# cbg-ethz/metMHN

Measured on AMD Instinct MI355X. Metric: full-cohort log-lik+grad evals/sec at n=20 events; kronvec HBM GB/s, higher is better.
Workload: dtype f64

## Files before the change

metmhn_amd/csrc/engine.hip:

```cpp
#include <algorithm>
#include <chrono>
#include <cmath>
#include <cstdio>
#include <cstdlib>
#include <cstring>
#include <string>
#include <vector>

#include "../../include/metmhn_amd.h"
#include "host.h"
#include "comm.h"
#include "plan.h"
#include "sampler.h"
#include "rowmix.h"

namespace mmhn {

static thread_local std::string g_err;

struct CListDev {
  DevArr<CItem> items;
  DevArr<int> deps;
};
struct StagedDev {
  DevArr<int> pats, paired, probs;
  DevArr<int2> map, lmap, grc;
  CListDev cl[2];
};
struct BatchDev {
  DevArr<PatRec> pats;
  DevArr<Desc> dJ, dS;
  DevArr<int2> mapJ, mapS, lmapJ, mapX, grcJ, lmapT;
  DevArr<int> sp_list[3][SP_NCLASS], paired, olist, ptoff;
  DevArr<uint32_t> ptiles;
  DevArr<WDesc> wd;
  DevArr<WChain> wchains;
  DevArr<int4> pcl;
  DevArr<double> wrow;
  CListDev clJ[2];
  StagedDev stg[2];
};

struct Config {
  PlanCfg plan;
  bool zero_copy = true;
  bool poison = false;
  bool force_timing = false;
  bool coop_fault = false;
  int coop_wgs = 0;
  bool coop = true;
  long long sim_chunk = 1ll << 26;
  int stream_blocks = 256 * 8;
  bool trace_host = false;
  Config() {
    plan.use_jacobi = env_is("MMHN_SOLVER", "jacobi");
    plan.psolve_min = (int)env_int("MMHN_PSOLVE_MIN", plan.psolve_min);
    plan.wsolve_min = (int)env_int("MMHN_WSOLVE_MIN", env_set("MMHN_PSOLVE_MIN") ? plan.psolve_min : plan.wsolve_min);
    plan.wsolve_mode = (int)env_int("MMHN_WSOLVE", plan.wsolve_mode);
    plan.wsolve_wgs = (int)env_int("MMHN_WSOLVE_WGS", plan.wsolve_wgs);
    plan.prep_split_max = (int)env_int("MMHN_PREP_SPLIT", plan.prep_split_max);
    plan.pcl_per = std::max(1, (int)env_int("MMHN_PCL_PER", plan.pcl_per));
    plan.small_path = env_flag("MMHN_SMALL", plan.small_path);
    zero_copy = env_flag("MMHN_ZEROCOPY", zero_copy);
    poison = env_flag("MMHN_POISON", poison);
    force_timing = env_flag("MMHN_TIME_KERNELS", force_timing);
    coop_fault = env_flag("MMHN_COOP_FAULT", coop_fault);
    coop_wgs = (int)env_int("MMHN_COOP_WGS", coop_wgs);
    coop = env_flag("MMHN_COOP", coop);
    sim_chunk = std::max(1ll, env_int("MMHN_SIM_CHUNK", sim_chunk));
    stream_blocks = (int)env_int("MMHN_STREAM_BLOCKS", stream_blocks);
    trace_host = env_set("MMHN_TRACE_HOST");
  }
};

struct EngineBase {
  virtual ~EngineBase() = default;
  int dtype = 0;
  int device = 0;
  hipStream_t stream = nullptr;
  Config cfg;
};

template <typename T> struct Engine;
template <typename T> void clear_row_groups(Engine<T>& E);
template <typename T> void launch_mix(Engine<T>& E, const Lane& L);
// ... 29 lines not shown
  std::vector<Batch> batches;
  std::vector<BatchDev> dev;
  DevArr<T> pi, lidgJ, qJ, rhsJ, rhsS, pS, lidgS, qS, seedS, GS, dots, bmJ, bmS, tabJ, tabS;
  DevArr<T> piM, qM;
  DevArr<T> zarena;
  struct View { T* p = nullptr; } GJ, DJ, Abuf;
  int pi_owner = -1, qJ_owner = -1;
  DevArr<double> lp, out, sums, abi_sums, redbuf;
  DevArr<double> resp;
  long long n_unknown = 0;
  std::vector<double> row_w;
  std::vector<long long> grp_ptr;
  std::vector<int> grp_rows;
  std::vector<double> grp_w;
  struct GroupsDev {
    DevArr<long long> gptr, mptr;
    DevArr<int> grows, mgrp;
    DevArr<double> gw, lpc, lpg, omega, lambda, rho;
  } gd;
  bool want_rho = false;
  DevArr<JLink<T>> links;
  double* h_abi = nullptr;
  double* h_abi_dev = nullptr;
  Lane main, side[3];
  DevArr<CoopCtl> coop_ctl;
  DevArr<unsigned> coop_flags[2];
  unsigned coop_epoch = 0;
  int coop_slot = 0;
  unsigned* h_abort = nullptr;
  unsigned* h_abort_dev = nullptr;
  bool coop_used = false;
  bool coop_alone = false;
  bool sums_pending = false;
  std::chrono::steady_clock::time_point sums_t0, sums_issued;
  int sums_len = 0;
  int pack_mode = 0;
  double pack_a = 0, pack_b = 0;
  double* pack_dst = nullptr;
  bool packed_in_eval = false;
  double reduce_flag = 0.0, reduce_flag_sum = 0.0;
  bool flag_pending = false;
  ncclComm_t comm = nullptr;
  int comm_rank = 0, comm_size = 1;
  bool time_kernels = true;
  mmhn_counters cnt{};
  std::vector<std::pair<hipEvent_t, hipEvent_t>> ev_pool;
  size_t ev_used = 0;
// ... 33 lines not shown
            if (popc(x) == l) perm[((size_t)t << TB) + pos++] = (uint16_t)x;
        }
        lvl[(size_t)t * (TB + 2) + t + 1] = pos;
      }
      d_perm.alloc(perm.size());
      d_lvl.alloc(lvl.size());
      HIPCHECK(hipMemcpy(d_perm.p, perm.data(), perm.size() * sizeof(uint16_t), hipMemcpyHostToDevice));
      HIPCHECK(hipMemcpy(d_lvl.p, lvl.data(), lvl.size() * sizeof(int), hipMemcpyHostToDevice));
    }
    raise_lds(wsolve_lds<T>(), &k_wsolve<T, false>, &k_wsolve<T, true>, &k_wsolve<T, false, WCfg<T>::NXT>, &k_wsolve<T, true, WCfg<T>::NXT>);
    raise_lds(wclass_lds<T>(), &k_wclass<T>);
    raise_lds(160 * 1024, &k_spatient2<T>, &k_spatient<T, 1024, 1>);
    raise_lds(150 * 1024,
              &k_csolve<T, false, false>, &k_csolve<T, true, false>, &k_csolve<T, false, true>, &k_csolve<T, true, true>,
              &k_csolve<T, false, false, 4>, &k_csolve<T, true, false, 4>,
              &k_psolve2<T, false, true>, &k_psolve2<T, true, true>, &k_psolve2<T, false, false>, &k_psolve2<T, true, false>,
              &k_tsolve<T, false, false>, &k_tsolve<T, true, false>, &k_tsolve<T, false, true>, &k_tsolve<T, true, true>,
              &k_kv<T, false, 1, false>, &k_kv<T, true, 1, false>, &k_kv<T, false, 1, true>, &k_kv<T, true, 1, true>,
              &k_sweep<T, false>, &k_sweep<T, true>, &k_diag<T>, &k_diag<T, 1024>,
              &k_prep<T, false>, &k_prep<T, true>, &k_prep<T, false, 1024>, &k_grad_rows<T, 1>, &k_grad_rows<T>,
              &k_pclass<T, false>, &k_pclass<T, true>, &k_class_marg<T>);
    coop_ctl.alloc(1);
    HIPCHECK(hipMemset(coop_ctl.p, 0, sizeof(CoopCtl)));
    HIPCHECK(hipHostMalloc(reinterpret_cast<void**>(&h_abort), 64, hipHostMallocDefault));
    HIPCHECK(hipHostGetDevicePointer(reinterpret_cast<void**>(&h_abort_dev), h_abort, 0));
    *h_abort = 0u;
    for (Lane& l : side) {
      HIPCHECK(hipStreamCreateWithFlags(&l.s, hipStreamNonBlocking));
      HIPCHECK(hipEventCreateWithFlags(&l.ev_fork, hipEventDisableTiming));
      HIPCHECK(hipEventCreateWithFlags(&l.ev_join, hipEventDisableTiming));
    }
    side[2].flags = 1;
  }
  ~Engine() override {
    comm_destroy();
    for (auto& e : ev_pool) { (void)hipEventDestroy(e.first); (void)hipEventDestroy(e.second); }
    for (Lane& l : side) {
      if (l.ev_join) (void)hipEventDestroy(l.ev_join);
      if (l.ev_fork) (void)hipEventDestroy(l.ev_fork);
      if (l.s) (void)hipStreamDestroy(l.s);
    }
    if (h_par) (void)hipHostFree(h_par);
    if (h_abi) (void)hipHostFree(h_abi);
    if (h_abort) (void)hipHostFree(h_abort);
    if (stream) (void)hipStreamDestroy(stream);
    stream = nullptr;
// ... 121 lines not shown
      launch();
      HIPCHECK(hipGetLastError());
      return;
    }
    if (ev_used == ev_pool.size()) {
      hipEvent_t a, b;
      HIPCHECK(hipEventCreate(&a));
      HIPCHECK(hipEventCreate(&b));
      ev_pool.push_back({a, b});
    }
    hipEvent_t e0 = ev_pool[ev_used].first, e1 = ev_pool[ev_used].second;
    ++ev_used;
    ev_bytes.push_back(alg_bytes);
    ev_slot.push_back(slot);
    HIPCHECK(hipEventRecord(e0, L.s));
    launch();
    HIPCHECK(hipGetLastError());
    HIPCHECK(hipEventRecord(e1, L.s));
  }

  size_t psolve2_lds(int maxk) const {
    return DESC_PAD + ((size_t)(1 << TB) + (size_t)((1 << TB) / TSB) + 3 * (size_t)maxk * 64 + (size_t)maxk * maxk + maxk) * sizeof(T) + 400 * sizeof(uint32_t) + (size_t)TSB * sizeof(uint16_t);
  }
  void psolve(const Lane& L, bool tr, const Batch& b, T* y, int rhs_mode) {
    const int nJ = (int)b.dJ.size();
    if (nJ == 0) return;
    const BatchDev& db = dev[b.id];
    if (b.wpath) {
      const int nW = (int)b.wd.size();
      double bytes = 0;
      for (const WDesc& w : b.wd) bytes += 0.5 * (double)(1ll << b.dJ[w.prob].k) * sizeof(T);
      T* yw = b.wdirect ? y : (tr ? qM.p : piM.p);
      timed(L, tr ? MMHN_K_PSOLVE_ADJ : MMHN_K_PSOLVE_FWD, bytes, [&]() {
        const int nch = (int)b.wchains.size();
        const dim3 g((unsigned)std::min(nch, cfg.plan.wsolve_wgs > 0 ? cfg.plan.wsolve_wgs : cfg.plan.n_cu)), bk(WROWS);
        const size_t lds = wsolve_lds<T>();
#define WS_ARGS g, bk, lds, L.s, db.dJ.p, db.wd.p, db.wchains.p, nch, yw, tabJ.p, links.p, qS.p
        if (b.wnx == WCfg<T>::NXT) { if (tr) hipLaunchKernelGGL((k_wsolve<T, true, WCfg<T>::NXT>), WS_ARGS); else hipLaunchKernelGGL((k_wsolve<T, false, WCfg<T>::NXT>), WS_ARGS); }
        else if (tr) hipLaunchKernelGGL((k_wsolve<T, true>), WS_ARGS);
        else hipLaunchKernelGGL((k_wsolve<T, false>), WS_ARGS);
#undef WS_ARGS
      });
      if (!b.wdirect) {
        hipLaunchKernelGGL((k_wconvert<T>), dim3(nW, 32), dim3(WROWS), 0, L.s, db.dJ.p, db.wd.p, yw, y);
        HIPCHECK(hipGetLastError());
      }
    }
    if (!b.olist.empty()) {
      const int mk = std::max(b.maxkP, 1);
      const long long spare = (80 * 1024 - 64) - (long long)psolve2_lds(mk);
      const int dl_cap = (int)std::max<long long>(0, std::min<long long>(PS_DL2, spare / (long long)sizeof(T)));
      const size_t lds = psolve2_lds(mk) + (size_t)dl_cap * sizeof(T);
      const double bytes = (double)b.ptiles.size() * (double)(1 << TB) * sizeof(T);
      const bool dlok = b.max_dl <= dl_cap;
      const int nold = (int)b.olist.size();
      timed(L, tr ? MMHN_K_PSOLVE_ADJ : MMHN_K_PSOLVE_FWD, bytes, [&]() {
        with_flags([&](auto tr_, auto dl) {
          hipLaunchKernelGGL((k_psolve2<T, tr_(), dl()>), dim3(nold), dim3(TSB), lds, L.s, db.dJ.p, db.ptoff.p, db.ptiles.p, d_par.p, y, rhs_mode,
                             d_perm.p, mk, tabJ.p, links.p, qS.p, dl_cap, db.olist.p);
        }, tr, dlok);
      });
    }
    if (!b.lmapT.empty()) {
      const PList LT{db.dJ.p, nullptr, (int)b.lmapT.size(), b.maxkT, 0, db.lmapT.p, &b.lofT, tabJ.p, b.clJ, db.clJ,
                     tr ? MMHN_K_CSOLVE_ADJ : MMHN_K_CSOLVE_FWD};
      solve(L, tr, LT, y, nullptr, nullptr, rhs_mode, nullptr);
    }
  }
// ... 54 lines not shown
                             d_perm.p, d_lvl.p, mk, P.tab, links.p, qS.p);
        }, tr, lidg != nullptr);
      });
    }
  }
  void check_abort() {
    if (!coop_used) return;
    coop_used = false;
    if (*h_abort == 0u) return;
    *h_abort = 0u;
    (void)hipMemset(coop_ctl.p, 0, sizeof(CoopCtl));
    throw Fail{"cooperative tile solve: a wait for another workgroup's tile timed out (results discarded)"};
  }

  void upload(const Batch& b, BatchDev& d) {
    auto up = [](auto& to, const auto& host) {
      if (host.empty()) return;
      to.alloc(host.size());
      HIPCHECK(hipMemcpy(to.p, host.data(), host.size() * sizeof(host[0]), hipMemcpyHostToDevice));
    };
    auto up_clist = [&](CListDev& to, const CList& cl) { up(to.items, cl.items); up(to.deps, cl.deps); };
    up(d.pats, b.pats); up(d.dJ, b.dJ); up(d.dS, b.dS);
    up(d.mapJ, b.mapJ); up(d.mapS, b.mapS); up(d.lmapJ, b.lmapJ); up(d.mapX, b.mapX); up(d.grcJ, b.grcJ);
    up(d.wd, b.wd); up(d.wchains, b.wchains); up(d.olist, b.olist); up(d.ptoff, b.ptoff); up(d.ptiles, b.ptiles);
    up(d.lmapT, b.lmapT); up_clist(d.clJ[0], b.clJ[0]); up_clist(d.clJ[1], b.clJ[1]);
    up(d.pcl, b.pcl); up(d.paired, b.paired);
    for (int w = 0; w < 3; ++w) for (int c = 0; c < SP_NCLASS; ++c) up(d.sp_list[w][c], b.sp_list[w][c]);
    for (int w = 0; w < 2; ++w) {
      const Staged& g = b.stg[w];
      StagedDev& dg = d.stg[w];
      up(dg.pats, g.pats); up(dg.paired, g.paired); up(dg.probs, g.probs);
      up(dg.map, g.map); up(dg.lmap, g.lmap); up(dg.grc, g.grc);
      up_clist(dg.cl[0], g.cl[0]); up_clist(dg.cl[1], g.cl[1]);
    }
  }
  void set_cohort(const int8_t* d_, long long np, int nc) {
    REQUIRE(nc == 2 * n + 3, "dat must have 2*n_mut+3 columns");
    REQUIRE(np >= 0, "negative patient count");
    REQUIRE(!sums_pending, "mmhn_set_cohort: an evaluation begun with mmhn_cohort_sums_begin has not been collected");
    dat.assign(d_, d_ + np * nc);
    n_pat = np;
    n_cols = nc;
    batches.clear();
    dev.clear();
    row_w.clear();
    clear_row_groups(*this);
    n_unknown = 0;
// ... 156 lines not shown
    const Staged& g = b.stg[w];
    const StagedDev& dg = db.stg[w];
    if (g.empty()) return;
    solve(L, true, staged_list(b, w), qS.p, lidgS.p, nullptr, 1, seedS.p);
    launch_grad_rows(L, db.dS.p, (int)g.probs.size(), g.maxk, nullptr, pS.p, qS.p, GS.p, GK_S, dg.grc);
    if (g.kind2) {
      hipLaunchKernelGGL((k_bit_marg<T>), dim3((unsigned)g.map.size()), dim3(BLOCK), 0, L.s, db.dS.p, dg.map.p, d_par.p, pS.p, qS.p, bmS.p);
      HIPCHECK(hipGetLastError());
    }
  }
  void joint_adjoint(const Batch& b) {
    const BatchDev& db = dev[b.id];
    if (cfg.plan.use_jacobi) zero(main, rhsJ.p, b.vecJ);
    for (int part = 0; part < 2 && !b.stg[1].paired.empty(); ++part) {
      if (b.stg[1].paired.size() >= 256)
        hipLaunchKernelGGL((k_scatter_marg<T, 1024>), dim3((unsigned)b.stg[1].paired.size()), dim3(1024), 0, main.s, db.pats.p, db.dJ.p,
                           db.dS.p, d_par.p, qS.p, rhsS.p, cfg.plan.use_jacobi ? rhsJ.p : nullptr, dots.p, part, db.stg[1].paired.p);
      else
        hipLaunchKernelGGL((k_scatter_marg<T>), dim3((unsigned)b.stg[1].paired.size()), dim3(BLOCK), 0, main.s, db.pats.p, db.dJ.p,
                           db.dS.p, d_par.p, qS.p, rhsS.p, cfg.plan.use_jacobi ? rhsJ.p : nullptr, dots.p, part, db.stg[1].paired.p);
      HIPCHECK(hipGetLastError());
    }
    if (cfg.plan.use_jacobi) solve(main, true, joint_list(b), qJ.p, lidgJ.p, rhsJ.p, 0, nullptr);
    else psolve(main, true, b, qJ.p, 3);
  }
  void joint_gradient(const Batch& b) {
    const BatchDev& db = dev[b.id];
    const int nJ = (int)b.dJ.size();
    if (!cfg.plan.use_jacobi) {
      const double mbytes = (double)b.vecJ * sizeof(T);
      timed(main, MMHN_K_PCLASS, mbytes, [&]() {
        if (b.wdirect) {
          const int nW = (int)b.wd.size();
          hipLaunchKernelGGL((k_wclass<T>), dim3((unsigned)std::min(nW, cfg.plan.n_cu)), dim3(WROWS), wclass_lds<T>(), main.s, db.dJ.p, db.wd.p, nW, pi.p, qJ.p, Abuf.p);
        }
        if (!b.pcl.empty())
          hipLaunchKernelGGL((k_pclass<T, true>), dim3((unsigned)b.pcl.size()), dim3(CMB), PC_LDS_ELEMS * sizeof(T), main.s, db.dJ.p, db.wd.p, pi.p, qJ.p, Abuf.p, db.pcl.p);
        else if ((int)b.wd.size() < nJ || !b.wdirect)
          hipLaunchKernelGGL((k_pclass<T, false>), dim3(nJ), dim3(CMB), PC_LDS_ELEMS * sizeof(T), main.s, db.dJ.p, db.wd.p, pi.p, qJ.p, Abuf.p);
      });
      if (!b.mapX.empty())
        hipLaunchKernelGGL((k_class_marg<T>), dim3((unsigned)b.mapX.size()), dim3(CMB), 2 * sizeof(T) << TB, main.s,
                           db.dJ.p, db.mapX.p, pi.p, qJ.p, Abuf.p);
    } else {
      hipLaunchKernelGGL((k_class_marg<T>), dim3((unsigned)b.mapJ.size()), dim3(CMB), 2 * sizeof(T) << TB, main.s, db.dJ.p,
                         db.mapJ.p, pi.p, qJ.p, Abuf.p);
    }
    HIPCHECK(hipGetLastError());
    if (b.pcl.empty()) {
      hipLaunchKernelGGL((k_eq_flows<T>), dim3(nJ), dim3(BLOCK), 0, main.s, db.dJ.p, db.wd.p, pi.p, qJ.p, Abuf.p);
      HIPCHECK(hipGetLastError());
    }
    launch_grad_rows(main, db.dJ.p, nJ, b.maxkcJ, Abuf.p, nullptr, nullptr, GJ.p, -1, db.grcJ, DJ.p, (long long)nJ * N * N);
  }
  void finalize_batch(const Batch& b, bool grad, bool gather) {
    const BatchDev& db = dev[b.id];
    const int npat = (int)b.pats.size(), nJ = (int)b.dJ.size();
    const AsmArgs<T> aa{db.pats.p, db.dJ.p, db.dS.p, d_par.p, GS.p, GJ.p, (long long)nJ * N * N, dots.p, DJ.p, (long long)nJ * N, bmS.p, lp.p, N,
// ... 965 lines not shown
```

metmhn_amd/csrc/plan.h:

```cpp
#pragma once
#include <algorithm>
#include <cmath>
#include <cstdint>
#include <string>
#include <vector>

#include "host.h"
#include "kernels.h"
#include "tsolve.h"
#include "small.h"
#include "wsolve.h"
#include "wclass.h"

namespace mmhn {

struct PlanCfg {
  size_t ws_limit = 0;
  int n_cu = 256;
  bool use_jacobi = false;
  int wsolve_mode = 1;
  int wsolve_min = 128;
  int psolve_min = 384;
  int wsolve_wgs = 0;
  int prep_split_max = 2048;
  int pcl_per = 16;
  bool small_path = true;
};

struct CList {
  std::vector<CItem> items;
  std::vector<int> deps;
  int maxk = 0;
  int nlevels = 0;
  void clear() { items.clear(); deps.clear(); maxk = 0; nlevels = 0; }
};
enum Route : uint8_t { RT_W = 0, RT_P = 1, RT_T = 2 };

struct Staged {
  std::vector<int> pats, paired, probs;
  std::vector<int2> map, lmap;
  std::vector<int> lof;
  std::vector<int2> grc;
  CList cl[2];
  int maxk = 0;
  bool kind2 = false;
  bool empty() const { return pats.empty(); }
};

struct Batch {
// ... 1 lines not shown
  std::vector<Desc> dJ, dS;
  std::vector<int2> mapJ, mapS;
  long long vecJ = 0, vecS = 0, asize = 0, tabJ = 0, tabS = 0;
  long long aclr = 0;
  int id = 0;
  int maxkJ = 0;
  int maxkcJ = 0;
  std::vector<int2> lmapJ;
  std::vector<int> lofJ;
  std::vector<int2> mapX;
  std::vector<int2> grcJ;
  std::vector<int> sp_list[3][SP_NCLASS];
  bool has_small = false;
  int mk1p = 9;
  Staged stg[2];
  std::vector<int> paired;
  std::vector<uint8_t> route;
  std::vector<int> olist;
  bool wpath = false;
  bool wdirect = false;
  std::vector<WDesc> wd;
  int wnx = -1;
  std::vector<WChain> wchains;
  long long offT = 0;
  CList clJ[2];
  std::vector<int2> lmapT;
  std::vector<int> lofT;
  int maxkT = 0, maxkP = 0;
  int max_dl = 0;
  std::vector<int> ptoff;
  std::vector<uint32_t> ptiles;
  std::vector<int4> pcl;
};

inline long long up4(long long v) { return (v + 3) / 4 * 4; }

static bool dead_tile(const Desc& d, uint32_t H) {
  if (d.mode != JOINT || d.seedbit < TB) return false;
  const uint32_t xhi = H << TB, hmask = ~((1u << TB) - 1u);
  if (xhi & (1u << d.seedbit)) return false;
  if (xhi & d.lone & hmask) return true;
  const uint32_t pp = d.pairP & hmask & ~(1u << 31);
  const uint32_t pm = (pp << 1);
  if (((xhi & pp) << 1) != (xhi & pm)) return true;
  return false;
}
// ... 266 lines not shown
template <typename T>
static void route_joint_problems(const PlanCfg& c, Batch& b) {
  const int nJ = (int)b.dJ.size();
  auto is_multi = [](const Desc& dj) { return dj.seedbit >= TB && popc(dj.pairP) <= TB; };
  b.route.assign((size_t)nJ, RT_T);
  b.olist.clear(); b.wd.clear(); b.wchains.clear();
  b.wpath = false;
  if (c.use_jacobi || nJ == 0) return;
  int nW = 0, nP = 0;
  if (c.wsolve_mode != 0) for (const Desc& dj : b.dJ) nW += window_ok<T>(dj) ? 1 : 0;
  b.wpath = nW > 0 && nW >= c.wsolve_min;
  for (int pj = 0; pj < nJ; ++pj) {
    if (b.wpath && window_ok<T>(b.dJ[pj])) b.route[pj] = RT_W;
    else if (is_multi(b.dJ[pj])) ++nP;
  }
  if (nP > 0 && nP >= c.psolve_min)
    for (int pj = 0; pj < nJ; ++pj) if (b.route[pj] != RT_W && is_multi(b.dJ[pj])) b.route[pj] = RT_P;
  for (int pj = 0; pj < nJ; ++pj) {
    if (b.route[pj] == RT_W) b.wd.push_back(make_wdesc<T>(b.dJ[pj], pj));
    else if (b.route[pj] == RT_P) b.olist.push_back(pj);
  }
}

static void layout_joint_vectors(Batch& b) {
  const int nJ = (int)b.dJ.size();
  std::stable_sort(b.wd.begin(), b.wd.end(), [](const WDesc& x, const WDesc& y) { return x.kR != y.kR ? x.kR < y.kR : x.kC < y.kC; });
  long long off = 0;
  for (const WDesc& w : b.wd) { b.dJ[w.prob].off = off; off += 1ll << b.dJ[w.prob].k; }
  for (int pj : b.olist) { b.dJ[pj].off = off; off += 1ll << b.dJ[pj].k; }
  b.offT = off;
  for (int pj = 0; pj < nJ; ++pj) if (b.route[pj] == RT_T) { b.dJ[pj].off = off; off += 1ll << b.dJ[pj].k; }
  REQUIRE(off == b.vecJ, "offsets of the joint problems do not add up");
}

template <typename T>
static void build_window_chains(const PlanCfg& c, Batch& b) {
  if (!b.wpath) return;
  const int nW = (int)b.wd.size();
  b.wnx = b.wd[0].nXc + b.wd[0].nXr;
  for (const WDesc& w : b.wd) if (w.nXc + w.nXr != b.wnx) b.wnx = -1;
  const int groups = std::max(1, c.wsolve_wgs > 0 ? c.wsolve_wgs : c.n_cu);
  const int per = (nW + groups - 1) / groups;
  for (int i0 = 0; i0 < nW;) {
    const WDesc& w = b.wd[i0];
    const int k = b.dJ[w.prob].k;
    const int maxlen = w.nXc + w.nXr >= 3 ? (int)std::min<long long>(per, (1ll << 31) / ((long long)sizeof(T) << k) - 1) : 1;
    int len = 1;
    while (len < maxlen && i0 + len < nW && b.wd[i0 + len].kR == w.kR && b.wd[i0 + len].kC == w.kC && (i0 + len) % per != 0) ++len;
    b.wchains.push_back(WChain{i0, len});
    i0 += len;
  }
  if ((int)b.wchains.size() <= groups) return;
  std::vector<WChain> srt = b.wchains;
  std::stable_sort(srt.begin(), srt.end(), [](const WChain& x, const WChain& y) { return x.count > y.count; });
  std::vector<std::vector<WChain>> mine((size_t)groups);
  std::vector<int> load((size_t)groups, 0);
  for (const WChain& ch : srt) {
    const int g = (int)(std::min_element(load.begin(), load.end()) - load.begin());
    mine[g].push_back(ch);
    load[g] += ch.count;
  }
  size_t rounds = 0;
  for (const auto& m : mine) rounds = std::max(rounds, m.size());
  b.wchains.assign(rounds * (size_t)groups, WChain{0, 0});
  for (int g = 0; g < groups; ++g)
    for (size_t r = 0; r < mine[g].size(); ++r) b.wchains[r * (size_t)groups + g] = mine[g][r];
}

static void build_tile_route(const PlanCfg& c, Batch& b) {
  b.lmapT.clear(); b.lofT.clear(); b.maxkT = 0;
  b.clJ[0].clear(); b.clJ[1].clear();
  if (c.use_jacobi) return;
  std::vector<int2> mt;
  for (const int2& m : b.mapJ) if (b.route[m.x] == RT_T) { mt.push_back(m); b.maxkT = std::max(b.maxkT, b.dJ[m.x].k); }
  if (mt.empty()) return;
  build_levels(mt, &b.dJ, true, b.lmapT, b.lofT);
  if (b.lofT.size() > 2) { build_clist(mt, b.dJ, true, false, b.clJ[0]); build_clist(mt, b.dJ, true, true, b.clJ[1]); }
}

static void build_psolve_tiles(Batch& b) {
  const int nJ = (int)b.dJ.size();
  b.ptoff.assign(1, 0);
  b.ptiles.clear();
  b.maxkP = 0; b.max_dl = 0;
  for (int pj = 0; pj < nJ; ++pj) {
    const Desc& dj = b.dJ[pj];
    if (b.route[pj] == RT_P) {
      const uint32_t nt = 1u << (dj.k - TB);
      for (uint32_t Ht = 0; Ht < nt; ++Ht) if (((Ht << TB) >> dj.seedbit) & 1u) b.ptiles.push_back(Ht);
// ... 113 lines not shown
  b.wdirect = b.wpath && c.wsolve_mode != 2;
  long long ao = 0;
  for (int pj = 0; pj < nJ; ++pj) if (!(b.wdirect && b.route[pj] == RT_W)) { b.dJ[pj].aoff = ao; ao += a_size(b.dJ[pj]); }
  b.aclr = up4(ao);
  ao = b.aclr;
  for (int pj = 0; pj < nJ; ++pj) if (b.wdirect && b.route[pj] == RT_W) { b.dJ[pj].aoff = ao; ao += a_size(b.dJ[pj]); }
  b.asize = ao;
  for (Desc& dj : b.dJ) dj.wl = -1;
  if (b.wdirect) for (size_t i = 0; i < b.wd.size(); ++i) b.dJ[b.wd[i].prob].wl = (int)i;
}

static void build_grad_chunks(Batch& b) {
  b.grcJ.clear();
  for (int kd = 0; kd < 3; ++kd)
    for (const int2& e : grad_chunks(b.dJ, kd)) b.grcJ.push_back(int2{e.x, e.y | (kd << 24)});
}

template <typename T>
static std::vector<Batch> plan_cohort(const PlanCfg& c, const int8_t* dat, long long np, int nc, int n, double& n_em) {
  const int N = n + 1;
  std::vector<Batch> batches = split_into_batches<T>(c, dat, np, nc, n, n_em);
  for (Batch& b : batches) {
    route_joint_problems<T>(c, b);
    layout_joint_vectors(b);
    build_window_chains<T>(c, b);
    build_tile_route(c, b);
    build_psolve_tiles(b);
    build_pclass_items(c, b);
    build_index_lists(c, b);
    assign_small_classes<T>(c, N, b);
    build_staged_groups(c, b);
    layout_class_arrays(c, b);
    build_grad_chunks(b);
  }
  return batches;
}

}
```

metmhn_amd/csrc/wclass.h:

```cpp
#pragma once
#include "kernels.h"

namespace mmhn {

template <typename T>
struct WClass {
  static constexpr int CHE = 32768 / (int)sizeof(T);
  static constexpr int LGCHE = sizeof(T) == 8 ? 12 : 13;
  static constexpr int LGMINR = 2;
  static constexpr int MX = WCfg<T>::KR - WTB < LGCHE - LGMINR - WCfg<T>::RB - WCfg<T>::HB ? WCfg<T>::KR - WTB
                                                                                           : LGCHE - LGMINR - WCfg<T>::RB - WCfg<T>::HB;
  static constexpr int XP = MX * (CHE >> (WCfg<T>::RB + WCfg<T>::HB));
  static constexpr size_t lds = (4 * (size_t)CHE + 2 * (size_t)XP) * sizeof(T) + WROWS * sizeof(uint16_t) + 64;
  static_assert((1 << LGCHE) == CHE, "");
};
template <typename T>
__host__ __device__ inline int wclass_mbits(int kC, int nXr) {
  const int m = WClass<T>::LGCHE - WClass<T>::LGMINR - kC;
  return m < 0 ? 0 : m < nXr ? m : nXr;
}
template <typename T>
__device__ __forceinline__ T seg_sum(T v, int lg) {
  if (lg > 0) v = dpp_stage<0>(v);
  if (lg > 1) v = dpp_stage<1>(v);
  if (lg > 2) v = dpp_stage<2>(v);
  if (lg > 3) v = dpp_stage<3>(v);
  if (lg > 4) v = dpp_stage<4>(v);
  if (lg > 5) v = dpp_stage<5>(v);
  return v;
}
template <typename T>
constexpr size_t wclass_lds() { return WClass<T>::lds; }

template <typename T>
__global__ __launch_bounds__(WROWS) void k_wclass(const Desc* __restrict__ descs, const WDesc* __restrict__ wds, int nw,
                                                  const T* __restrict__ p, const T* __restrict__ q, T* A) {
  using C = WCfg<T>;
  constexpr int RB = C::RB, HB = C::HB, NC = 1 << RB, H = 1 << HB, KC = C::KC, WNXR = C::KR - WTB;
  constexpr int QE = 16 / (int)sizeof(T), LGQ = QE == 2 ? 1 : 2, NQ = NC / QE;
  constexpr int CHE = WClass<T>::CHE;
  typedef T VecT __attribute__((ext_vector_type(NC)));
  typedef T QT __attribute__((ext_vector_type(QE)));
  static_assert(NQ == 2 && CHE == WROWS * NC, "a block row is two 16-byte pieces; a block fills one staged array");
  extern __shared__ __align__(16) unsigned char smem[];
  T* const lds = reinterpret_cast<T*>(smem);
  const int tid = threadIdx.x;
  const uint32_t rho = wrho((uint32_t)tid >> 6, (uint32_t)tid & 63u);
  uint16_t* const rinv = reinterpret_cast<uint16_t*>(lds + 4 * (size_t)CHE + 2 * (size_t)WClass<T>::XP);
  rinv[rho] = (uint16_t)tid;
  for (int it = blockIdx.x; it < nw; it += gridDim.x) {
    const WDesc& wd = wds[it];
    const Desc& d = descs[wd.prob];
    const int k = d.k, kR = wd.kR, kC = wd.kC, nXc = wd.nXc, nXr = wd.nXr;
    const bool majP = wd.majP != 0;
    const long long half = 1ll << (k - 1);
    const T* ps = p + d.off + half;
    const T* qs = q + d.off + half;
    const int kP = __popc(d.maskP);
    T* outR = A + d.aoff + (majP ? 0 : class_block_size(kP));
    T* outC = A + d.aoff + (majP ? class_block_size(kP) : 0);
    const int NBc = (1 << nXc) << HB;
    const int mX = wclass_mbits<T>(kC, nXr);
    auto ldv = [&](const T* src, uint32_t Sigma, uint32_t beta, uint32_t row) -> VecT {
      const QT* a = reinterpret_cast<const QT*>(src + wpos<T>(Sigma, beta, row, 0));
      const QT lo = a[0], hi = a[1];
      VecT v;
#pragma unroll
      for (int e = 0; e < QE; ++e) { v[e] = lo[e]; v[QE + e] = hi[e]; }
      return v;
    };
    auto dot = [&](const VecT& a, const VecT& b) -> T {
      T s = a[0] * b[0];
#pragma unroll
      for (int c = 1; c < NC; ++c) s += a[c] * b[c];
      return s;
    };
    __syncthreads();
    for (uint32_t Sx = 0; Sx < (1u << nXr); ++Sx) {
      T acc[1 + WTB + WNXR];
#pragma unroll
      for (int s = 0; s < 1 + WTB + WNXR; ++s) acc[s] = T(0);
      VecT pn = ldv(ps, Sx << nXc, 0, rho), qn = ldv(qs, Sx << nXc, 0, rho);
      for (int B = 0; B < NBc; ++B) {
        const uint32_t Sigma = ((uint32_t)B >> HB) | (Sx << nXc), beta = (uint32_t)B & (uint32_t)(H - 1);
        const VecT pv = pn, qv = qn;
        if (B + 1 < NBc) {
          const uint32_t Sg2 = ((uint32_t)(B + 1) >> HB) | (Sx << nXc), b2 = (uint32_t)(B + 1) & (uint32_t)(H - 1);
          pn = ldv(ps, Sg2, b2, rho); qn = ldv(qs, Sg2, b2, rho);
        }
        T* qb = lds + (B & 1) * CHE;
        {
          QT lo, hi;
#pragma unroll
          for (int e = 0; e < QE; ++e) { lo[e] = qv[e]; hi[e] = qv[QE + e]; }
          *reinterpret_cast<QT*>(qb + (size_t)tid * QE) = lo;
          *reinterpret_cast<QT*>(qb + (size_t)(WROWS + tid) * QE) = hi;
        }
        __syncthreads();
        acc[0] -= dot(pv, qv);
#pragma unroll
        for (int i = 0; i < WTB; ++i) {
          const uint32_t nb = (uint32_t)tid | (1u << i);
          const QT lo = *reinterpret_cast<const QT*>(qb + (size_t)nb * QE);
          const QT hi = *reinterpret_cast<const QT*>(qb + (size_t)(WROWS + nb) * QE);
          T s = T(0);
#pragma unroll
          for (int e = 0; e < QE; ++e) s += pv[e] * lo[e] + pv[QE + e] * hi[e];
          acc[1 + i] += s;
        }
#pragma unroll
        for (int i = 0; i < WNXR; ++i) {
          if (i >= mX && i < nXr && !((Sx >> i) & 1u)) {
            const VecT qx = ldv(qs, Sigma | (1u << (nXc + i)), beta, rho);
            acc[1 + WTB + i] += dot(pv, qx);
          }
        }
      }
      const long long S = (long long)tid | ((long long)Sx << WTB);
      outR[S] = acc[0];
#pragma unroll
      for (int i = 0; i < WTB; ++i)
        if (!((tid >> i) & 1)) outR[((long long)(1 + i) << kR) + S] = acc[1 + i];
#pragma unroll
      for (int i = 0; i < WNXR; ++i)
        if (i >= mX && i < nXr && !((Sx >> i) & 1u)) outR[((long long)(1 + WTB + i) << kR) + S] = acc[1 + WTB + i];
    }
    {
      constexpr int XP = WClass<T>::XP, JU = sizeof(T) == 8 ? 2 : 1;
      static_assert(CHE == 2 * WROWS * QE, "a thread takes two rows of a chunk");
      const int lgR = WClass<T>::LGCHE - kC - mX;
      const int RCH = 1 << lgR, RCX = RCH << mX;
      const int lgnch = WTB - lgR, nch = 1 << lgnch;
      const int lgP = kC - LGQ, NPc = 1 << lgP;
      const int cp = tid & (NPc - 1);
      const int r0 = tid >> lgP, rstep = WROWS >> lgP;
      const int lgRX = lgR + mX, nW = lgP > 6 ? 1 << (lgP - 6) : 1;
      T* const xpart = lds + 4 * (size_t)CHE;
      T ac[QE][1 + KC];
#pragma unroll
      for (int e = 0; e < QE; ++e)
#pragma unroll
        for (int s = 0; s <= KC; ++s) ac[e][s] = T(0);
      const int lgrl = lgR + 1;
      auto piece_src = [&](int g, uint32_t sxh, int ch) -> long long {
        const int run = g >> lgrl, rr = g & ((1 << lgrl) - 1);
        const uint32_t Sigma = ((uint32_t)run >> HB) | (sxh << (nXc + mX)), beta = (uint32_t)run & (uint32_t)(H - 1);
        return wpos<T>(Sigma, beta, (uint32_t)(ch * RCH + (rr >> 1)), (uint32_t)((rr & 1) * QE));
      };
      auto piece_dst = [&](int g) -> int {
        const int run = g >> lgrl, rr = g & ((1 << lgrl) - 1);
// ... 7 lines not shown
      auto xfinish = [&](int cidx) {
        const T* xp = xpart + (cidx & 1) * XP;
        for (int i = tid; i < (mX << lgRX); i += WROWS) {
          const int l = i >> lgRX, r = i & (RCX - 1);
          if (!((r >> (lgR + l)) & 1)) {
            T v = xp[(size_t)i * nW];
            for (int w = 1; w < nW; ++w) v += xp[(size_t)i * nW + w];
            outR[((long long)(1 + WTB + l) << kR) + row_S(cidx, r)] = v;
          }
        }
      };
      const int ntot = nch << (nXr - mX);
      QT rp[2], rq[2];
      auto fetch = [&](int cidx) {
        const uint32_t sxh = (uint32_t)(cidx >> lgnch);
        const int ch = cidx & (nch - 1);
#pragma unroll
        for (int j = 0; j < 2; ++j) {
          const long long src = piece_src(tid + WROWS * j, sxh, ch);
          rp[j] = *reinterpret_cast<const QT*>(ps + src);
          rq[j] = *reinterpret_cast<const QT*>(qs + src);
        }
      };
      __syncthreads();
      fetch(0);
      for (int cidx = 0; cidx < ntot; ++cidx) {
        T* pc = lds + (size_t)(2 * (cidx & 1)) * CHE;
        T* qc = pc + CHE;
#pragma unroll
        for (int j = 0; j < 2; ++j) {
          const int dst = piece_dst(tid + WROWS * j);
          *reinterpret_cast<QT*>(pc + dst) = rp[j];
          *reinterpret_cast<QT*>(qc + dst) = rq[j];
        }
        if (cidx + 1 < ntot) fetch(cidx + 1);
        __syncthreads();
        if (mX > 0 && cidx > 0) xfinish(cidx - 1);
#pragma unroll JU
        for (int j = 0; j < 2; ++j) {
          const int r = r0 + j * rstep;
          const T* prow = pc + ((size_t)r << kC);
          const T* qrow = qc + ((size_t)r << kC);
          const QT pv = *reinterpret_cast<const QT*>(prow + cp * QE);
          const QT qv = *reinterpret_cast<const QT*>(qrow + cp * QE);
#pragma unroll
          for (int e = 0; e < QE; ++e) ac[e][0] -= pv[e] * qv[e];
#pragma unroll
// ... 50 lines not shown
```

Baseline: 22.68.

## Split window-solve remainder onto side lane and ticket-schedule wclass work items

When the number of window problems leaves a small remainder over the workgroup count, the cheapest eligible remainder problems are split off into a separate batch B. Its solve runs on a fourth side stream concurrently with the main batch, and its gradient class work also runs on that side stream. The wclass kernel is reworked to pull work items (row half or column half of a problem) from an atomic ticket counter, with items sorted most expensive first. This targets the tail imbalance where a few leftover problems idle most CUs. In exchange it adds atomic contention, extra launches and stream fork/join overhead, and it reorders the planning steps.

```diff
diff --git a/metmhn_amd/csrc/engine.hip b/metmhn_amd/csrc/engine.hip
--- a/metmhn_amd/csrc/engine.hip
+++ b/metmhn_amd/csrc/engine.hip
@@ -35,6 +35,7 @@
   DevArr<uint32_t> ptiles;
   DevArr<WDesc> wd;
   DevArr<WChain> wchains;
+  DevArr<int2> wcl;
   DevArr<int4> pcl;
   DevArr<double> wrow;
   CListDev clJ[2];
@@ -61,6 +62,7 @@
     plan.prep_split_max = (int)env_int("MMHN_PREP_SPLIT", plan.prep_split_max);
     plan.pcl_per = std::max(1, (int)env_int("MMHN_PCL_PER", plan.pcl_per));
     plan.small_path = env_flag("MMHN_SMALL", plan.small_path);
+    plan.wrem = env_flag("MMHN_WREM", true);
     zero_copy = env_flag("MMHN_ZEROCOPY", zero_copy);
     poison = env_flag("MMHN_POISON", poison);
     force_timing = env_flag("MMHN_TIME_KERNELS", force_timing);
@@ -136,7 +138,8 @@
   DevArr<JLink<T>> links;
   double* h_abi = nullptr;
   double* h_abi_dev = nullptr;
-  Lane main, side[3];
+  Lane main, side[4];
+  DevArr<unsigned> wtick;
   DevArr<CoopCtl> coop_ctl;
   DevArr<unsigned> coop_flags[2];
   unsigned coop_epoch = 0;
@@ -216,6 +219,8 @@
               &k_pclass<T, false>, &k_pclass<T, true>, &k_class_marg<T>);
     coop_ctl.alloc(1);
     HIPCHECK(hipMemset(coop_ctl.p, 0, sizeof(CoopCtl)));
+    wtick.alloc(2);
+    HIPCHECK(hipMemset(wtick.p, 0, 2 * sizeof(unsigned)));
     HIPCHECK(hipHostMalloc(reinterpret_cast<void**>(&h_abort), 64, hipHostMallocDefault));
     HIPCHECK(hipHostGetDevicePointer(reinterpret_cast<void**>(&h_abort_dev), h_abort, 0));
     *h_abort = 0u;
@@ -383,28 +388,39 @@
   size_t psolve2_lds(int maxk) const {
     return DESC_PAD + ((size_t)(1 << TB) + (size_t)((1 << TB) / TSB) + 3 * (size_t)maxk * 64 + (size_t)maxk * maxk + maxk) * sizeof(T) + 400 * sizeof(uint32_t) + (size_t)TSB * sizeof(uint16_t);
   }
-  void psolve(const Lane& L, bool tr, const Batch& b, T* y, int rhs_mode) {
+  void wsolve_part(const Lane& L, bool tr, const Batch& b, T* y, int w0, int nw, int c0, int nch) {
+    const BatchDev& db = dev[b.id];
+    double bytes = 0;
+    for (int i = w0; i < w0 + nw; ++i) bytes += 0.5 * (double)(1ll << b.dJ[b.wd[i].prob].k) * sizeof(T);
+    T* yw = b.wdirect ? y : (tr ? qM.p : piM.p);
+    timed(L, tr ? MMHN_K_PSOLVE_ADJ : MMHN_K_PSOLVE_FWD, bytes, [&]() {
+      const dim3 g((unsigned)std::min(nch, cfg.plan.wsolve_wgs > 0 ? cfg.plan.wsolve_wgs : cfg.plan.n_cu)), bk(WROWS);
+      const size_t lds = wsolve_lds<T>();
+#define WS_ARGS g, bk, lds, L.s, db.dJ.p, db.wd.p, db.wchains.p + c0, nch, yw, tabJ.p, links.p, qS.p
+      if (b.wnx == WCfg<T>::NXT) { if (tr) hipLaunchKernelGGL((k_wsolve<T, true, WCfg<T>::NXT>), WS_ARGS); else hipLaunchKernelGGL((k_wsolve<T, false, WCfg<T>::NXT>), WS_ARGS); }
+      else if (tr) hipLaunchKernelGGL((k_wsolve<T, true>), WS_ARGS);
+      else hipLaunchKernelGGL((k_wsolve<T, false>), WS_ARGS);
+#undef WS_ARGS
+    });
+    if (!b.wdirect) {
+      hipLaunchKernelGGL((k_wconvert<T>), dim3(nw, 32), dim3(WROWS), 0, L.s, db.dJ.p, db.wd.p + w0, yw, y);
+      HIPCHECK(hipGetLastError());
+    }
+  }
+  void wsolve_A(const Lane& L, bool tr, const Batch& b, T* y) { wsolve_part(L, tr, b, y, 0, b.nwA, 0, b.nchA); }
+  void wsolve_B(const Lane& L, bool tr, const Batch& b, T* y) {
+    wsolve_part(L, tr, b, y, b.nwA, (int)b.wd.size() - b.nwA, b.nchA, (int)b.wchains.size() - b.nchA);
+  }
+  static bool wsplit(const Batch& b) { return b.wpath && b.nwA < (int)b.wd.size(); }
+  void psolve(const Lane& L, bool tr, const Batch& b, T* y, int rhs_mode, Lane* rem = nullptr) {
     const int nJ = (int)b.dJ.size();
     if (nJ == 0) return;
     const BatchDev& db = dev[b.id];
     if (b.wpath) {
-      const int nW = (int)b.wd.size();
-      double bytes = 0;
-      for (const WDesc& w : b.wd) bytes += 0.5 * (double)(1ll << b.dJ[w.prob].k) * sizeof(T);
-      T* yw = b.wdirect ? y : (tr ? qM.p : piM.p);
-      timed(L, tr ? MMHN_K_PSOLVE_ADJ : MMHN_K_PSOLVE_FWD, bytes, [&]() {
-        const int nch = (int)b.wchains.size();
-        const dim3 g((unsigned)std::min(nch, cfg.plan.wsolve_wgs > 0 ? cfg.plan.wsolve_wgs : cfg.plan.n_cu)), bk(WROWS);
-        const size_t lds = wsolve_lds<T>();
-#define WS_ARGS g, bk, lds, L.s, db.dJ.p, db.wd.p, db.wchains.p, nch, yw, tabJ.p, links.p, qS.p
-        if (b.wnx == WCfg<T>::NXT) { if (tr) hipLaunchKernelGGL((k_wsolve<T, true, WCfg<T>::NXT>), WS_ARGS); else hipLaunchKernelGGL((k_wsolve<T, false, WCfg<T>::NXT>), WS_ARGS); }
-        else if (tr) hipLaunchKernelGGL((k_wsolve<T, true>), WS_ARGS);
-        else hipLaunchKernelGGL((k_wsolve<T, false>), WS_ARGS);
-#undef WS_ARGS
-      });
-      if (!b.wdirect) {
-        hipLaunchKernelGGL((k_wconvert<T>), dim3(nW, 32), dim3(WROWS), 0, L.s, db.dJ.p, db.wd.p, yw, y);
-        HIPCHECK(hipGetLastError());
+      wsolve_A(L, tr, b, y);
+      if (wsplit(b)) {
+        if (rem) rem->begin(L);
+        wsolve_B(rem ? *rem : L, tr, b, y);
       }
     }
     if (!b.olist.empty()) {
@@ -505,7 +521,7 @@
     auto up_clist = [&](CListDev& to, const CList& cl) { up(to.items, cl.items); up(to.deps, cl.deps); };
     up(d.pats, b.pats); up(d.dJ, b.dJ); up(d.dS, b.dS);
     up(d.mapJ, b.mapJ); up(d.mapS, b.mapS); up(d.lmapJ, b.lmapJ); up(d.mapX, b.mapX); up(d.grcJ, b.grcJ);
-    up(d.wd, b.wd); up(d.wchains, b.wchains); up(d.olist, b.olist); up(d.ptoff, b.ptoff); up(d.ptiles, b.ptiles);
+    up(d.wd, b.wd); up(d.wchains, b.wchains); up(d.wcl, b.wcl); up(d.olist, b.olist); up(d.ptoff, b.ptoff); up(d.ptiles, b.ptiles);
     up(d.lmapT, b.lmapT); up_clist(d.clJ[0], b.clJ[0]); up_clist(d.clJ[1], b.clJ[1]);
     up(d.pcl, b.pcl); up(d.paired, b.paired);
     for (int w = 0; w < 3; ++w) for (int c = 0; c < SP_NCLASS; ++c) up(d.sp_list[w][c], b.sp_list[w][c]);
@@ -708,18 +724,35 @@
       HIPCHECK(hipGetLastError());
     }
     if (cfg.plan.use_jacobi) solve(main, true, joint_list(b), qJ.p, lidgJ.p, rhsJ.p, 0, nullptr);
-    else psolve(main, true, b, qJ.p, 3);
+    else psolve(main, true, b, qJ.p, 3, &side[3]);
   }
   void joint_gradient(const Batch& b) {
     const BatchDev& db = dev[b.id];
     const int nJ = (int)b.dJ.size();
     if (!cfg.plan.use_jacobi) {
-      const double mbytes = (double)b.vecJ * sizeof(T);
+      double mbytes = (double)b.vecJ * sizeof(T);
+      auto wclass = [&](const Lane& L, int part, int i0, int ni, int wgs, int drawers) {
+        hipLaunchKernelGGL((k_wclass<T>), dim3((unsigned)wgs), dim3(WROWS), wclass_lds<T>(), L.s, db.dJ.p, db.wd.p,
+                           db.wcl.p + i0, ni, wtick.p + part, (unsigned)drawers, pi.p, qJ.p, Abuf.p);
+      };
+      Lane& rem = side[3];
+      const int niA = 2 * b.nwA, niB = (int)b.wcl.size() - niA;
+      const int wgA = std::max(std::min(niA, cfg.plan.n_cu), rem.forked ? 2 : 1);
+      const int wgB = rem.forked ? std::max(1, std::min({niB / 2, cfg.plan.n_cu / 2, wgA - 1})) : 0;
+      if (rem.forked) {
+        if (b.wdirect) {
+          double bytesB = 0;
+          for (size_t i = (size_t)b.nwA; i < b.wd.size(); ++i) bytesB += (double)(1ll << b.dJ[b.wd[i].prob].k) * sizeof(T);
+          mbytes -= bytesB;
+          timed(rem, MMHN_K_PCLASS, bytesB, [&]() { wclass(rem, 1, niA, niB, wgB, wgB); });
+          wclass(rem, 0, 0, niA, wgB, wgA);
+          HIPCHECK(hipGetLastError());
+        }
+        rem.end();
+      }
       timed(main, MMHN_K_PCLASS, mbytes, [&]() {
-        if (b.wdirect) {
-          const int nW = (int)b.wd.size();
-          hipLaunchKernelGGL((k_wclass<T>), dim3((unsigned)std::min(nW, cfg.plan.n_cu)), dim3(WROWS), wclass_lds<T>(), main.s, db.dJ.p, db.wd.p, nW, pi.p, qJ.p, Abuf.p);
-        }
+        if (b.wdirect) wclass(main, 0, 0, niA, wgA - wgB, wgA);
+        rem.join(main);
         if (!b.pcl.empty())
           hipLaunchKernelGGL((k_pclass<T, true>), dim3((unsigned)b.pcl.size()), dim3(CMB), PC_LDS_ELEMS * sizeof(T), main.s, db.dJ.p, db.wd.p, pi.p, qJ.p, Abuf.p, db.pcl.p);
         else if ((int)b.wd.size() < nJ || !b.wdirect)
diff --git a/metmhn_amd/csrc/plan.h b/metmhn_amd/csrc/plan.h
--- a/metmhn_amd/csrc/plan.h
+++ b/metmhn_amd/csrc/plan.h
@@ -25,6 +25,7 @@
   int prep_split_max = 2048;
   int pcl_per = 16;
   bool small_path = true;
+  bool wrem = false;
 };
 
 struct CList {
@@ -72,6 +73,9 @@
   std::vector<WDesc> wd;
   int wnx = -1;
   std::vector<WChain> wchains;
+  int nwA = 0, nchA = 0;
+  int nspB = 0;
+  std::vector<int2> wcl;
   long long offT = 0;
   CList clJ[2];
   std::vector<int2> lmapT;
@@ -384,9 +388,31 @@
   }
 }
 
-static void layout_joint_vectors(Batch& b) {
+static void split_window_remainder(const PlanCfg& c, Batch& b) {
+  const int nW = (int)b.wd.size();
+  b.nwA = nW; b.nspB = 0;
+  if (!b.wpath || !c.wrem) return;
+  const int groups = std::max(1, c.wsolve_wgs > 0 ? c.wsolve_wgs : c.n_cu);
+  const int r = nW % groups;
+  if (nW < 2 * groups || r == 0 || r > groups / 2) return;
+  std::vector<int> pat_of(b.dJ.size(), -1);
+  for (size_t pi_ = 0; pi_ < b.pats.size(); ++pi_) if (b.pats[pi_].j >= 0) pat_of[b.pats[pi_].j] = (int)pi_;
+  std::vector<char> elig(b.pats.size(), 0), inB(b.pats.size(), 0);
+  for (int pi_ : b.sp_list[1][2]) elig[pi_] = 1;
+  std::vector<int> cand;
+  for (int i = 0; i < nW; ++i) if (pat_of[b.wd[i].prob] >= 0 && elig[pat_of[b.wd[i].prob]]) cand.push_back(i);
+  if ((int)cand.size() < r) return;
+  std::stable_sort(cand.begin(), cand.end(), [&](int x, int y) { return b.dJ[b.wd[x].prob].k < b.dJ[b.wd[y].prob].k; });
+  for (int i = 0; i < r; ++i) inB[pat_of[b.wd[cand[i]].prob]] = 1;
+  std::stable_partition(b.wd.begin(), b.wd.end(), [&](const WDesc& w) { return !inB[pat_of[w.prob]]; });
+  std::stable_partition(b.sp_list[1][2].begin(), b.sp_list[1][2].end(), [&](int pi_) { return !inB[pi_]; });
+  b.nwA = nW - r; b.nspB = r;
+}
+
+static void layout_joint_vectors(const PlanCfg& c, Batch& b) {
   const int nJ = (int)b.dJ.size();
   std::stable_sort(b.wd.begin(), b.wd.end(), [](const WDesc& x, const WDesc& y) { return x.kR != y.kR ? x.kR < y.kR : x.kC < y.kC; });
+  split_window_remainder(c, b);
   long long off = 0;
   for (const WDesc& w : b.wd) { b.dJ[w.prob].off = off; off += 1ll << b.dJ[w.prob].k; }
   for (int pj : b.olist) { b.dJ[pj].off = off; off += 1ll << b.dJ[pj].k; }
@@ -402,16 +428,36 @@
   b.wnx = b.wd[0].nXc + b.wd[0].nXr;
   for (const WDesc& w : b.wd) if (w.nXc + w.nXr != b.wnx) b.wnx = -1;
   const int groups = std::max(1, c.wsolve_wgs > 0 ? c.wsolve_wgs : c.n_cu);
-  const int per = (nW + groups - 1) / groups;
-  for (int i0 = 0; i0 < nW;) {
-    const WDesc& w = b.wd[i0];
-    const int k = b.dJ[w.prob].k;
-    const int maxlen = w.nXc + w.nXr >= 3 ? (int)std::min<long long>(per, (1ll << 31) / ((long long)sizeof(T) << k) - 1) : 1;
-    int len = 1;
-    while (len < maxlen && i0 + len < nW && b.wd[i0 + len].kR == w.kR && b.wd[i0 + len].kC == w.kC && (i0 + len) % per != 0) ++len;
-    b.wchains.push_back(WChain{i0, len});
-    i0 += len;
-  }
+  auto cut = [&](int lo, int hi, int per) {
+    for (int i0 = lo; i0 < hi;) {
+      const WDesc& w = b.wd[i0];
+      const int k = b.dJ[w.prob].k;
+      const int maxlen = w.nXc + w.nXr >= 3 ? (int)std::min<long long>(per, (1ll << 31) / ((long long)sizeof(T) << k) - 1) : 1;
+      int len = 1;
+      while (len < maxlen && i0 + len < hi && b.wd[i0 + len].kR == w.kR && b.wd[i0 + len].kC == w.kC && (i0 + len - lo) % per != 0) ++len;
+      b.wchains.push_back(WChain{i0, len});
+      i0 += len;
+    }
+  };
+  if (b.nwA < nW) {
+    const int per = b.nwA / groups;
+    cut(0, b.nwA, per);
+    std::vector<std::vector<WChain>> mine((size_t)groups);
+    for (const WChain& ch : b.wchains) mine[ch.start / per].push_back(ch);
+    size_t rounds = 0;
+    for (auto& m : mine) {
+      std::stable_sort(m.begin(), m.end(), [](const WChain& x, const WChain& y) { return x.count > y.count; });
+      rounds = std::max(rounds, m.size());
+    }
+    b.wchains.assign(rounds * (size_t)groups, WChain{0, 0});
+    for (int g = 0; g < groups; ++g)
+      for (size_t r = 0; r < mine[g].size(); ++r) b.wchains[r * (size_t)groups + g] = mine[g][r];
+    b.nchA = (int)b.wchains.size();
+    cut(b.nwA, nW, 1);
+    return;
+  }
+  cut(0, nW, (nW + groups - 1) / groups);
+  b.nchA = (int)b.wchains.size();
   if ((int)b.wchains.size() <= groups) return;
   std::vector<WChain> srt = b.wchains;
   std::stable_sort(srt.begin(), srt.end(), [](const WChain& x, const WChain& y) { return x.count > y.count; });
@@ -427,6 +473,25 @@
   b.wchains.assign(rounds * (size_t)groups, WChain{0, 0});
   for (int g = 0; g < groups; ++g)
     for (size_t r = 0; r < mine[g].size(); ++r) b.wchains[r * (size_t)groups + g] = mine[g][r];
+  b.nchA = (int)b.wchains.size();
+}
+
+template <typename T>
+static void build_wclass_items(Batch& b) {
+  b.wcl.clear();
+  if (!b.wpath) return;
+  const int nW = (int)b.wd.size();
+  auto price = [&](const int2& it) -> long long {
+    const WDesc& w = b.wd[it.x];
+    const int extra = it.y == 0 ? w.nXr - wclass_mbits<T>(w.kC, w.nXr) : 0;
+    return (4ll + extra) << (b.dJ[w.prob].k - 1);
+  };
+  for (int i = 0; i < nW; ++i) { b.wcl.push_back(int2{i, 0}); b.wcl.push_back(int2{i, 1}); }
+  auto dearest_first = [&](int lo, int hi) {
+    std::stable_sort(b.wcl.begin() + lo, b.wcl.begin() + hi, [&](const int2& x, const int2& y) { return price(x) > price(y); });
+  };
+  dearest_first(0, 2 * b.nwA);
+  dearest_first(2 * b.nwA, 2 * nW);
 }
 
 static void build_tile_route(const PlanCfg& c, Batch& b) {
@@ -586,13 +651,14 @@
   std::vector<Batch> batches = split_into_batches<T>(c, dat, np, nc, n, n_em);
   for (Batch& b : batches) {
     route_joint_problems<T>(c, b);
-    layout_joint_vectors(b);
+    assign_small_classes<T>(c, N, b);
+    layout_joint_vectors(c, b);
     build_window_chains<T>(c, b);
+    build_wclass_items<T>(b);
     build_tile_route(c, b);
     build_psolve_tiles(b);
     build_pclass_items(c, b);
     build_index_lists(c, b);
-    assign_small_classes<T>(c, N, b);
     build_staged_groups(c, b);
     layout_class_arrays(c, b);
     build_grad_chunks(b);
diff --git a/metmhn_amd/csrc/wclass.h b/metmhn_amd/csrc/wclass.h
--- a/metmhn_amd/csrc/wclass.h
+++ b/metmhn_amd/csrc/wclass.h
@@ -33,7 +33,8 @@
 constexpr size_t wclass_lds() { return WClass<T>::lds; }
 
 template <typename T>
-__global__ __launch_bounds__(WROWS) void k_wclass(const Desc* __restrict__ descs, const WDesc* __restrict__ wds, int nw,
+__global__ __launch_bounds__(WROWS) void k_wclass(const Desc* __restrict__ descs, const WDesc* __restrict__ wds,
+                                                  const int2* __restrict__ items, int nitems, unsigned* ticket, unsigned drawers,
                                                   const T* __restrict__ p, const T* __restrict__ q, T* A) {
   using C = WCfg<T>;
   constexpr int RB = C::RB, HB = C::HB, NC = 1 << RB, H = 1 << HB, KC = C::KC, WNXR = C::KR - WTB;
@@ -48,8 +49,18 @@
   const uint32_t rho = wrho((uint32_t)tid >> 6, (uint32_t)tid & 63u);
   uint16_t* const rinv = reinterpret_cast<uint16_t*>(lds + 4 * (size_t)CHE + 2 * (size_t)WClass<T>::XP);
   rinv[rho] = (uint16_t)tid;
-  for (int it = blockIdx.x; it < nw; it += gridDim.x) {
-    const WDesc& wd = wds[it];
+  __shared__ unsigned s_item;
+  for (;;) {
+    __syncthreads();
+    if (tid == 0) s_item = atomicAdd(ticket, 1u);
+    __syncthreads();
+    const unsigned it = s_item;
+    if (it >= (unsigned)nitems) {
+      if (tid == 0 && it == (unsigned)nitems + drawers - 1u) __hip_atomic_store(ticket, 0u, __ATOMIC_RELAXED, __HIP_MEMORY_SCOPE_AGENT);
+      break;
+    }
+    const int2 item = items[it];
+    const WDesc& wd = wds[item.x];
     const Desc& d = descs[wd.prob];
     const int k = d.k, kR = wd.kR, kC = wd.kC, nXc = wd.nXc, nXr = wd.nXr;
     const bool majP = wd.majP != 0;
@@ -75,57 +86,58 @@
       for (int c = 1; c < NC; ++c) s += a[c] * b[c];
       return s;
     };
-    __syncthreads();
-    for (uint32_t Sx = 0; Sx < (1u << nXr); ++Sx) {
-      T acc[1 + WTB + WNXR];
-#pragma unroll
-      for (int s = 0; s < 1 + WTB + WNXR; ++s) acc[s] = T(0);
-      VecT pn = ldv(ps, Sx << nXc, 0, rho), qn = ldv(qs, Sx << nXc, 0, rho);
-      for (int B = 0; B < NBc; ++B) {
-        const uint32_t Sigma = ((uint32_t)B >> HB) | (Sx << nXc), beta = (uint32_t)B & (uint32_t)(H - 1);
-        const VecT pv = pn, qv = qn;
-        if (B + 1 < NBc) {
-          const uint32_t Sg2 = ((uint32_t)(B + 1) >> HB) | (Sx << nXc), b2 = (uint32_t)(B + 1) & (uint32_t)(H - 1);
-          pn = ldv(ps, Sg2, b2, rho); qn = ldv(qs, Sg2, b2, rho);
-        }
-        T* qb = lds + (B & 1) * CHE;
-        {
-          QT lo, hi;
-#pragma unroll
-          for (int e = 0; e < QE; ++e) { lo[e] = qv[e]; hi[e] = qv[QE + e]; }
-          *reinterpret_cast<QT*>(qb + (size_t)tid * QE) = lo;
-          *reinterpret_cast<QT*>(qb + (size_t)(WROWS + tid) * QE) = hi;
-        }
-        __syncthreads();
-        acc[0] -= dot(pv, qv);
-#pragma unroll
-        for (int i = 0; i < WTB; ++i) {
-          const uint32_t nb = (uint32_t)tid | (1u << i);
-          const QT lo = *reinterpret_cast<const QT*>(qb + (size_t)nb * QE);
-          const QT hi = *reinterpret_cast<const QT*>(qb + (size_t)(WROWS + nb) * QE);
-          T s = T(0);
-#pragma unroll
-          for (int e = 0; e < QE; ++e) s += pv[e] * lo[e] + pv[QE + e] * hi[e];
-          acc[1 + i] += s;
-        }
-#pragma unroll
-        for (int i = 0; i < WNXR; ++i) {
-          if (i >= mX && i < nXr && !((Sx >> i) & 1u)) {
-            const VecT qx = ldv(qs, Sigma | (1u << (nXc + i)), beta, rho);
-            acc[1 + WTB + i] += dot(pv, qx);
-          }
-        }
+    if (item.y == 0) {
+      for (uint32_t Sx = 0; Sx < (1u << nXr); ++Sx) {
+        T acc[1 + WTB + WNXR];
+#pragma unroll
+        for (int s = 0; s < 1 + WTB + WNXR; ++s) acc[s] = T(0);
+        VecT pn = ldv(ps, Sx << nXc, 0, rho), qn = ldv(qs, Sx << nXc, 0, rho);
+        for (int B = 0; B < NBc; ++B) {
+          const uint32_t Sigma = ((uint32_t)B >> HB) | (Sx << nXc), beta = (uint32_t)B & (uint32_t)(H - 1);
+          const VecT pv = pn, qv = qn;
+          if (B + 1 < NBc) {
+            const uint32_t Sg2 = ((uint32_t)(B + 1) >> HB) | (Sx << nXc), b2 = (uint32_t)(B + 1) & (uint32_t)(H - 1);
+            pn = ldv(ps, Sg2, b2, rho); qn = ldv(qs, Sg2, b2, rho);
+          }
+          T* qb = lds + (B & 1) * CHE;
+          {
+            QT lo, hi;
+#pragma unroll
+            for (int e = 0; e < QE; ++e) { lo[e] = qv[e]; hi[e] = qv[QE + e]; }
+            *reinterpret_cast<QT*>(qb + (size_t)tid * QE) = lo;
+            *reinterpret_cast<QT*>(qb + (size_t)(WROWS + tid) * QE) = hi;
+          }
+          __syncthreads();
+          acc[0] -= dot(pv, qv);
+#pragma unroll
+          for (int i = 0; i < WTB; ++i) {
+            const uint32_t nb = (uint32_t)tid | (1u << i);
+            const QT lo = *reinterpret_cast<const QT*>(qb + (size_t)nb * QE);
+            const QT hi = *reinterpret_cast<const QT*>(qb + (size_t)(WROWS + nb) * QE);
+            T s = T(0);
+#pragma unroll
+            for (int e = 0; e < QE; ++e) s += pv[e] * lo[e] + pv[QE + e] * hi[e];
+            acc[1 + i] += s;
+          }
+#pragma unroll
+          for (int i = 0; i < WNXR; ++i) {
+            if (i >= mX && i < nXr && !((Sx >> i) & 1u)) {
+              const VecT qx = ldv(qs, Sigma | (1u << (nXc + i)), beta, rho);
+              acc[1 + WTB + i] += dot(pv, qx);
+            }
+          }
+        }
+        const long long S = (long long)tid | ((long long)Sx << WTB);
+        outR[S] = acc[0];
+#pragma unroll
+        for (int i = 0; i < WTB; ++i)
+          if (!((tid >> i) & 1)) outR[((long long)(1 + i) << kR) + S] = acc[1 + i];
+#pragma unroll
+        for (int i = 0; i < WNXR; ++i)
+          if (i >= mX && i < nXr && !((Sx >> i) & 1u)) outR[((long long)(1 + WTB + i) << kR) + S] = acc[1 + WTB + i];
       }
-      const long long S = (long long)tid | ((long long)Sx << WTB);
-      outR[S] = acc[0];
-#pragma unroll
-      for (int i = 0; i < WTB; ++i)
-        if (!((tid >> i) & 1)) outR[((long long)(1 + i) << kR) + S] = acc[1 + i];
-#pragma unroll
-      for (int i = 0; i < WNXR; ++i)
-        if (i >= mX && i < nXr && !((Sx >> i) & 1u)) outR[((long long)(1 + WTB + i) << kR) + S] = acc[1 + WTB + i];
     }
-    {
+    else {
       constexpr int XP = WClass<T>::XP, JU = sizeof(T) == 8 ? 2 : 1;
       static_assert(CHE == 2 * WROWS * QE, "a thread takes two rows of a chunk");
       const int lgR = WClass<T>::LGCHE - kC - mX;
@@ -179,7 +191,6 @@
           rq[j] = *reinterpret_cast<const QT*>(qs + src);
         }
       };
-      __syncthreads();
       fetch(0);
       for (int cidx = 0; cidx < ntot; ++cidx) {
         T* pc = lds + (size_t)(2 * (cidx & 1)) * CHE;
```

After: 22.89, median of 6. No clear change (+0.9%).
